# edo01/2024-EUMaster4HPC-Student-Challenge

Measured on AMD Instinct MI355X. Metric: cg_iterations_per_sec, higher is better.
Workload: dtype f64

## Files before the change

### 2024-eumaster4hpc-student-challenge_amd/csrc/lam_ctx.h

```cpp
#pragma once

namespace {

thread_local std::string g_create_error;

double now_s()
{
    return std::chrono::duration<double>(std::chrono::steady_clock::now().time_since_epoch()).count();
}

uint64_t thread_cpu_ns()
{
    struct timespec ts;
    if (clock_gettime(CLOCK_THREAD_CPUTIME_ID, &ts) != 0) return 0;
    return (uint64_t)ts.tv_sec * 1000000000ull + (uint64_t)ts.tv_nsec;
}

constexpr int kLag = 4;
constexpr int64_t kRankModeDefaultExchange = 1;
constexpr int64_t kOneProcessDefaultExchange = 1;
constexpr int kVecBlocksMax = 256;

struct SymvDevPlan {
    SymvTask *tasks = nullptr;
// ... 113 lines not shown
    bool shifted = false;
    MshiftState ms;
    MinresState mr;
    SymvDevPlan sym;
    int sym_vec = 0, sym_cap_K = 0;
};

struct PcgState {
    void *diag = nullptr, *dinv = nullptr;
    double *part_rz = nullptr;
    DiagInfo *info = nullptr;
    uint64_t diag_gen = ~0ull;
    uint64_t bad_count = 0, bad_row = 0;
    double bad_value = 0.0;
    void *dinv_k = nullptr;
    uint64_t dinvk_gen = ~0ull;
    int dinvk_K = 0, dinvk_nrhs = 0;
    double dinvk_shift[kMaxRhs] = {};
    uint64_t badk_count = 0, badk_row = 0;
    int badk_col = 0;
    double badk_value = 0.0;
};

}

struct lam_hip_ctx {
    MultiState multi;
    PcgState pcg;
    int dtype = LAM_HIP_F64;
    int total_shards = 1;
    int rank = 0, nranks = 1;
    bool rank_mode = false;
    ncclComm_t comm = nullptr;
    double t_comm_init = 0.0;
    uint64_t n = 0;
    uint64_t lda = 0;
    bool have_problem = false, have_matrix = false, have_rhs = false, cg_ready = false;
    int k_done = 0;
    std::vector<ShardBase> sh;
    std::string err;
    int64_t opt_gemv_variant = -1;
    int64_t opt_nt = 1;
    int64_t opt_generic = 0;
    int64_t opt_probe_rows = 0;
    int64_t opt_overlap = 1;
    int64_t opt_panel_lo = 0, opt_panel_hi = 0;
    bool gather_pending = false;
    int64_t opt_symmetric_many = 0;
    bool symv_many_effective = false;
    int64_t opt_symmetric = 0;
    int64_t opt_exchange = 0;
// ... 21 lines not shown
    bool direct_ok = false;
    bool cg_direct = false;
    int64_t opt_verify_direct = 1;
    int64_t direct_fallbacks = 0;
    uint32_t epoch = 0;
    uint64_t seq_base = 0, seq_span = 1;
    int *direct_err = nullptr;
    double *agree_buf = nullptr;
    bool cg_exchange1 = false;
    double t_gemv_min = 0.0, t_gemv_max = 0.0;
    int xt_slot = -1;
    int ranks_on_device = 1;
    bool symmetric_from_env = false;
    uint64_t matrix_gen = 0, sym_checked_gen = ~0ull;
    bool sym_refused = false;
    bool told_sym_ineffective = false;

    bool symv_wanted() const
    {
        return n > 0 && !sym_refused && (opt_symmetric >= 2 || (opt_symmetric == 1 && n * n * (uint64_t)esz_a() >= (192ull << 20)));
    }
    bool symv_active() const { return symv_wanted() && !rank_mode && total_shards == 1; }
    bool symv_multi_active() const { return symv_wanted() && exchange1_ok(); }
    uint64_t symv_stride_bytes() const { return (n * esz_v() + 7) / 8 * 8 + 8; }

    bool exchange2_wanted() const { return (rank_mode || total_shards > 1) && opt_exchange == 2 && opt_finalize != 0; }
    bool exchange1_ok() const { return (rank_mode || total_shards > 1) && opt_exchange == 1 && n >= (uint64_t)total_shards; }
    uint64_t ex1_base() const { return n / (uint64_t)total_shards; }
    uint64_t ex1_maxrows() const { return n / (uint64_t)total_shards + n % (uint64_t)total_shards; }
    uint64_t ex1_stride_bytes() const { return (ex1_maxrows() * esz_v() + 7) / 8 * 8 + 8; }

    size_t esz_a() const { return dtype == LAM_HIP_F64 ? 8 : (dtype == LAM_HIP_F32 ? 4 : 2); }
    static uint64_t pitch_for(uint64_t n, size_t ea) { return lam::row_pitch(n, ea); }
    uint64_t ncols_vec() const { const uint64_t v = 16 / esz_a(); return (n + v - 1) / v * v; }
    size_t esz_v() const { return dtype == LAM_HIP_F64 ? 8 : 4; }
};

namespace {

int fail(lam_hip_ctx *c, int code, const char *fmt, ...)
{
    char buf[512];
    va_list ap;
    va_start(ap, fmt);
    vsnprintf(buf, sizeof buf, fmt, ap);
    va_end(ap);
// ... 148 lines not shown
```

### 2024-eumaster4hpc-student-challenge_amd/csrc/lam_hip.hip

```cpp
#include <hip/hip_runtime.h>
#include <rccl/rccl.h>

#include <algorithm>
#include <atomic>
#include <chrono>
#include <cmath>
#include <cstdarg>
#include <cstdio>
#include <cstdlib>
#include <cstring>
#include <memory>
#include <new>
#include <mutex>
#include <string>
#include <type_traits>
#include <vector>

#include <sched.h>
#include <time.h>
#include <unistd.h>

#include "../../include/lam_hip.h"
#include "lam_kernels.h"

// ... 111 lines not shown
        c->t_comm_init = now_s() - t0;
        rc = count_ranks_on_device(c.get());
        if (rc != 0) {
            g_create_error = c->err;
            (void)ncclCommDestroy(c->comm);
            c->comm = nullptr;
            abandon(c.get());
            return rc;
        }
    }
    *out = c.release();
    return 0;
}

void lam_hip_destroy(lam_hip_ctx *c)
{
    if (!c) return;
    for (auto &s : c->sh) {
        (void)hipSetDevice(s.dev);
        if (s.stream) (void)hipStreamSynchronize(s.stream);
    }
    multi_release(c);
    close_direct(c);
    if (c->agree_buf) (void)hipFree(c->agree_buf);
    for (auto &s : c->sh) {
        if (hipSetDevice(s.dev) != hipSuccess) { (void)hipGetLastError(); continue; }
        if (s.mail) { (void)hipFree(s.mail); s.mail = nullptr; }
        if (s.bcast) { (void)hipFree(s.bcast); s.bcast = nullptr; }
    }
    if (c->direct_err) (void)hipHostFree(c->direct_err);
    if (c->comm) (void)ncclCommDestroy(c->comm);
    release_join(c);
    for (auto &s : c->sh) {
        free_shard(s);
        release_handles(s);
    }
    delete c;
}

int lam_hip_set_problem(lam_hip_ctx *c, uint64_t n)
{
    if (!c) return LAM_HIP_EINVAL;
    if (n == 0) return fail(c, LAM_HIP_EINVAL, "n must be > 0");
    if (n < (uint64_t)c->total_shards) return fail(c, LAM_HIP_EINVAL, "n (%llu) smaller than the number of shards", (unsigned long long)n);
    if (n != c->multi.n) multi_release(c);
    c->multi.have_rhs = c->multi.solved = c->multi.ms.valid = c->multi.lz.valid = false;
    multi_clear_shifts(c->multi);
    c->n = n;
    c->iter_est_s = 0.0;
    c->lda = lam_hip_ctx::pitch_for(n, c->esz_a());
    c->problem_gen++;
    c->have_problem = c->have_matrix = c->have_rhs = c->cg_ready = false;
    const size_t ea = c->esz_a(), ev = c->esz_v();
    for (auto &s : c->sh) {
        free_shard(s, c->opt_reuse_matrix != 0);
        partition(n, c->total_shards, s.index, &s.row0, &s.nrows);
        LAMCHK(set_dev(c, s));
        const size_t needA = std::max<size_t>(16, s.nrows * c->lda * ea);
        if (s.A != nullptr && s.A_capacity < needA) { (void)hipFree(s.A); s.A = nullptr; s.A_capacity = 0; }
        if (s.A == nullptr) {
            HIPCHK(c, hipMalloc(&s.A, needA));
            s.A_capacity = needA;
        }
        HIPCHK(c, hipMalloc(&s.p, n * ev + 64));
        HIPCHK(c, hipMalloc(&s.tmp, n * ev + 64));
        void **vecs[] = {&s.Ap, &s.x, &s.r, &s.b};
        for (auto v : vecs) HIPCHK(c, hipMalloc(v, s.nrows * ev + 16));
        s.gemv_blocks = dispatch(c, [&](auto impl) -> int { return decltype(impl)::gemv_grid(c, s.nrows); });
        const int gemv_blocks_max = (int)std::max<uint64_t>(s.nrows, (n + kSymvReduceRows - 1) / kSymvReduceRows) + 1;
        s.vec_blocks = vec_grid(s.nrows);
        HIPCHK(c, hipMalloc((void **)&s.part_gemv, sizeof(double) * (size_t)gemv_blocks_max));
        s.part_gemv_cap = gemv_blocks_max;
        HIPCHK(c, hipMalloc((void **)&s.part_vec, sizeof(double) * kVecBlocksMax));
        HIPCHK(c, hipMalloc((void **)&s.part_aux, sizeof(double) * kVecBlocksMax));
        HIPCHK(c, hipMalloc((void **)&s.gather_a, sizeof(double) * kMaxShards));
// ... 322 lines not shown
    ShardBase &s0 = c->sh[0];
    c->prog_t = 0.0;
    IterTimes times;
    int enq = 0;
    LAMCHK(set_dev(c, s0));
    HIPCHK(c, hipMemcpyAsync(s0.sc_host, s0.sc, sizeof(CgScalars), hipMemcpyDeviceToHost, s0.stream));
    HIPCHK(c, hipStreamSynchronize(s0.stream));
    const bool stopped = s0.sc_host->stop != 0;
    const int k_first = c->k_done + 1;
    for (auto &sh_ : c->sh)
        for (int i = 0; i < kLag; i++) { sh_.timed_slot[i] = false; sh_.nx[i] = 0; }
    if (stopped) {
    } else {
        for (int i = 0; i < iters; i++) {
            const int k = k_first + i;
            const int slot = i % kLag;
            if (i >= kLag) {
                LAMCHK(set_dev(c, s0));
                const int d = lag_check(c, s0, k);
                if (d < 0) return d;
                if (d != 0) break;
                harvest_times(c, slot, &times);
            }
            const double te = now_s();
            LAMCHK(enqueue_iteration(c, k, rel_error, slot));
            c->enqueue_ns += (uint64_t)((now_s() - te) * 1e9);
            enq++;
        }
    }
    if (enq > 0) {
        Progress pr;
        LAMCHK(set_dev(c, s0));
        LAMCHK(await_progress(c, s0, k_first + enq - 1, &pr, true));
    }
    LAMCHK(settle_gather(c));
    LAMCHK(sync_all(c));
    if (*c->direct_err != 0) {
        static const char *what[] = {"", "", "a peer's partial dot product (direct exchange)", "a peer's p slice (direct exchange)",
                                     "the reducer workgroup's broadcast inside the fused update launch (its workgroups were not all resident?)",
                                     "a workgroup's partial inside a launch (reducer workgroup)"};
        const int code = c->direct_err[0];
        return fail(c, LAM_HIP_EHIP, "rank %d: a bounded in-kernel wait expired waiting for %s (code %d; slot %d, expected tag %d:%d, saw %d:%d); "
                                     "the iteration state is no longer valid", c->rank, code >= 2 && code <= 5 ? what[code] : "?", code,
                    c->direct_err[1], c->direct_err[4], c->direct_err[2], c->direct_err[5], c->direct_err[3]);
    }
    if (c->cg_direct && c->rank_mode && c->nranks > 1 && enq > 0) {
// ... 7 lines not shown
    const CgScalars sc = *s0.sc_host;
    c->k_done = sc.iters;
    const double t1 = now_s();
    if (st) {
        memset(st, 0, sizeof *st);
        const int ran = sc.iters - (k_first - 1);
        st->converged = sc.stop != 0;
        st->num_iters = sc.stop ? sc.iters : sc.iters + 1;
        st->rel_err = std::sqrt(sc.rr[sc.iters & 1] / sc.bb);
        st->t_total = t1 - t0;
        st->t_iter = ran > 0 ? (t1 - t0) / ran : 0.0;
        double tmin = 0.0, tmax = 0.0;
        for (size_t j = 0; j < c->sh.size(); j++) {
            if (times.samples[j] == 0) continue;
            const double avg = times.gemv_ms[j] * 1e-3 / times.samples[j];
            tmax = std::max(tmax, avg);
            tmin = tmin == 0.0 ? avg : std::min(tmin, avg);
        }
        c->t_gemv_min = tmin;
        c->t_gemv_max = tmax;
        st->t_gemv = tmax;
        st->t_exchange = times.samples[0] > 0 ? times.xch_ms * 1e-3 / times.samples[0] : 0.0;
        st->t_comm_init = c->t_comm_init;
        st->gemv_bytes = (double)c->esz_a() * (double)s0.nrows * (double)c->n + (double)c->esz_v() * (double)(c->n + s0.nrows);
    }
    (void)enq;
    return 0;
}

int lam_hip_solve(lam_hip_ctx *c, int max_iters, double rel_error, lam_hip_stats *st)
{
    if (!c) return LAM_HIP_EINVAL;
    if (max_iters < 0) return fail(c, LAM_HIP_EINVAL, "max_iters must be >= 0");
    const double t0 = now_s();
    lam_hip_stats local;
    LAMCHK(lam_hip_cg_init(c));
    LAMCHK(lam_hip_cg_iterate(c, max_iters, rel_error, &local));
    if (c->cg_direct && c->opt_verify_direct) {
        double tr = 0.0;
        LAMCHK(lam_hip_true_residual(c, &tr));
        const double slack = c->dtype == LAM_HIP_F64 ? 2.2e-10 : 1e-4;
        if (!(tr <= 10.0 * local.rel_err + slack)) {
            if (c->rank == 0)
                fprintf(stderr, "lam_hip: direct exchange: recomputed residual %.3e does not match the recursive residual %.3e -- "
                                "solving again on the RCCL exchange\n", tr, local.rel_err);
            c->direct_fallbacks++;
            c->opt_exchange = 0;
// ... 36 lines not shown
        HIPCHK(c, hipStreamSynchronize(s.stream));
    }
    return 0;
}

static int gemv_tmp(lam_hip_ctx *c)
{
    return dispatch(c, [&](auto impl) -> int {
        using I = decltype(impl);
        using TV = typename ImplTraits<I>::TV;
        for (auto &s : c->sh) {
            LAMCHK(set_dev(c, s));
            LAMCHK(I::launch_gemv(c, s, (const TV *)s.tmp, (TV *)s.Ap, nullptr, nullptr));
        }
        return 0;
    });
}

int lam_hip_gemv(lam_hip_ctx *c, const void *x_host, void *y_host)
{
    if (!c || !x_host || !y_host) return LAM_HIP_EINVAL;
    if (!c->have_matrix) return fail(c, LAM_HIP_ESTATE, "matrix not set");
    LAMCHK(env_symmetric_check(c));
    const size_t ev = c->esz_v();
    for (auto &s : c->sh) {
        LAMCHK(set_dev(c, s));
        HIPCHK(c, hipMemcpyAsync(s.tmp, x_host, c->n * ev, hipMemcpyHostToDevice, s.stream));
    }
    if (c->symv_active()) {
        LAMCHK(dispatch(c, [&](auto impl) -> int {
            using I = decltype(impl);
            using TV = typename ImplTraits<I>::TV;
            ShardBase &s = c->sh[0];
            LAMCHK(set_dev(c, s));
            return I::launch_symv(c, s, (const TV *)s.tmp, (TV *)s.Ap, nullptr, nullptr);
        }));
    } else {
        LAMCHK(gemv_tmp(c));
    }
    c->cg_ready = false;
    if (c->rank_mode) {
        ShardBase &s = c->sh[0];
        const ncclDataType_t dt = c->dtype == LAM_HIP_F64 ? ncclDouble : ncclFloat;
        HIPCHK(c, hipMemcpyAsync((char *)s.tmp + s.row0 * ev, s.Ap, s.nrows * ev, hipMemcpyDeviceToDevice, s.stream));
        NCCLCHK(c, ncclGroupStart());
        for (int q = 0; q < c->nranks; q++) {
// ... 1 lines not shown
            partition(c->n, c->nranks, q, &r0, &nr);
            char *ptr = (char *)s.tmp + r0 * ev;
            NCCLCHK(c, ncclBroadcast(ptr, ptr, nr, dt, q, c->comm, s.stream));
            c->n_collectives++;
        }
        NCCLCHK(c, ncclGroupEnd());
        HIPCHK(c, hipMemcpyAsync(y_host, s.tmp, c->n * ev, hipMemcpyDeviceToHost, s.stream));
        HIPCHK(c, hipStreamSynchronize(s.stream));
        return 0;
    }
    for (auto &s : c->sh) {
        LAMCHK(set_dev(c, s));
        HIPCHK(c, hipMemcpyAsync((char *)y_host + s.row0 * ev, s.Ap, s.nrows * ev, hipMemcpyDeviceToHost, s.stream));
        HIPCHK(c, hipStreamSynchronize(s.stream));
    }
    return 0;
}

int lam_hip_gemv_only(lam_hip_ctx *c, int reps, double *sec)
{
    if (!c || !sec || reps < 1) return LAM_HIP_EINVAL;
    if (!c->have_matrix) return fail(c, LAM_HIP_ESTATE, "matrix not set");
    LAMCHK(env_symmetric_check(c));
    c->cg_ready = false;
    double worst = 0.0;
    LAMCHK(dispatch(c, [&](auto impl) -> int {
        using I = decltype(impl);
        using TV = typename ImplTraits<I>::TV;
        for (auto &s : c->sh) {
            LAMCHK(set_dev(c, s));
            const uint64_t nrows_saved = s.nrows;
            if (c->opt_probe_rows > 0) s.nrows = std::min<uint64_t>(s.nrows, (uint64_t)c->opt_probe_rows);
            const bool split = c->opt_panel_hi > c->opt_panel_lo;
            const uint64_t lo = (uint64_t)c->opt_panel_lo, hi = (uint64_t)c->opt_panel_hi;
            auto one = [&]() -> int {
                if (c->symv_active()) return I::launch_symv(c, s, (const TV *)s.p, (TV *)s.Ap, s.part_gemv, nullptr);
                if (!split) return I::launch_gemv(c, s, (const TV *)s.p, (TV *)s.Ap, s.part_gemv, nullptr);
                int r1 = I::launch_gemv(c, s, (const TV *)s.p, (TV *)s.Ap, nullptr, nullptr, 1, lo, hi);
                return r1 != 0 ? r1 : I::launch_gemv(c, s, (const TV *)s.p, (TV *)s.Ap, s.part_gemv, nullptr, 2, lo, hi);
            };
            int rc = one();
            if (rc == 0 && hipEventRecord(s.ev_g0[0], s.stream) != hipSuccess) rc = LAM_HIP_EHIP;
            for (int i = 0; i < reps && rc == 0; i++) rc = one();
            if (rc == 0 && hipEventRecord(s.ev_g1[0], s.stream) != hipSuccess) rc = LAM_HIP_EHIP;
            s.nrows = nrows_saved;
            if (rc != 0) return rc == LAM_HIP_EHIP ? fail(c, rc, "hipEventRecord failed in gemv_only") : rc;
// ... 215 lines not shown
    else if (!strcmp(name, "exchange")) { c->opt_exchange = value; c->cg_ready = false; }
    else if (!strcmp(name, "exchange_join")) c->opt_join = value;
    else if (!strcmp(name, "finalize")) {
        if (value == 0 && !kTuningBuild)
            return fail(c, LAM_HIP_EINVAL, "finalize = 0 (separate reduction launches, the round-1 chain) exists in the tuning build only (`make tuning`, "
                                           "load liblam_hip_tuning.so through LAM_HIP_LIB), not in the product library");
        c->opt_finalize = value; c->cg_ready = false;
    }
    else if (!strcmp(name, "upload_staging")) c->opt_upload_staging = value;
    else if (!strcmp(name, "reuse_matrix")) c->opt_reuse_matrix = value;
    else if (!strcmp(name, "fuse_update")) { c->opt_fuse = value; c->cg_ready = false; }
    else if (!strcmp(name, "symmetric")) {
        c->opt_symmetric = value;
        c->symmetric_from_env = false;
        c->sym_refused = false;
        c->cg_ready = false;
    }
    else if (!strcmp(name, "symmetric_many")) {
        if (value < 0 || value > 2)
            return fail(c, LAM_HIP_EINVAL, "symmetric_many = %lld: 0 (general batched product), 1 (symmetric where it pays) or 2 (always, K <= 4)",
                        (long long)value);
        c->opt_symmetric_many = value;
    }
    else if (!strcmp(name, "gemv_timing")) c->opt_gemv_timing = value < 0 ? 0 : value;
    else if (!strcmp(name, "verify_direct")) c->opt_verify_direct = value;
    else if (!strcmp(name, "assume_cus")) { c->opt_assume_cus = value; c->cg_ready = false; }
    else if (!strcmp(name, "panel_lo")) c->opt_panel_lo = value;
    else if (!strcmp(name, "panel_hi")) c->opt_panel_hi = value;
    else return fail(c, LAM_HIP_EINVAL, "unknown option '%s'", name);
    for (auto &s : c->sh)
        if (c->have_problem) s.gemv_blocks = dispatch(c, [&](auto impl) -> int { return decltype(impl)::gemv_grid(c, s.nrows); });
    return 0;
}

int lam_hip_get_option(const lam_hip_ctx *c, const char *name, int64_t *value)
{
    if (!c || !name || !value) return LAM_HIP_EINVAL;
    if (!strcmp(name, "gemv_variant")) *value = c->opt_gemv_variant;
    else if (!strcmp(name, "nt_loads")) *value = c->opt_nt;
    else if (!strcmp(name, "force_generic")) *value = c->opt_generic;
    else if (!strcmp(name, "probe_rows")) *value = c->opt_probe_rows;
    else if (!strcmp(name, "overlap")) *value = c->opt_overlap;
    else if (!strcmp(name, "exchange")) *value = c->opt_exchange;
    else if (!strcmp(name, "exchange_join")) *value = c->opt_join;
    else if (!strcmp(name, "finalize")) *value = c->opt_finalize;
    else if (!strcmp(name, "upload_staging")) *value = c->opt_upload_staging;
// ... 3 lines not shown
    else if (!strcmp(name, "rccl_ranks")) {
        int count = 0;
        if (c->comm != nullptr && ncclCommCount(c->comm, &count) != ncclSuccess) count = -1;
        *value = count;
    }
    else if (!strcmp(name, "ranks_on_device")) *value = c->ranks_on_device;
    else if (!strcmp(name, "gemv_ns_min_shard")) *value = (int64_t)(c->t_gemv_min * 1e9);
    else if (!strcmp(name, "gemv_ns_max_shard")) *value = (int64_t)(c->t_gemv_max * 1e9);
    else if (!strcmp(name, "tuning_variants")) *value = kTuningBuild ? 1 : 0;
    else if (!strcmp(name, "fuse_effective")) *value = c->fuse_active ? 1 : 0;
    else if (!strcmp(name, "gemv_timing")) *value = c->opt_gemv_timing;
    else if (!strcmp(name, "verify_direct")) *value = c->opt_verify_direct;
    else if (!strcmp(name, "direct_fallbacks")) *value = c->direct_fallbacks;
    else if (!strcmp(name, "assume_cus")) *value = c->opt_assume_cus;
    else if (!strcmp(name, "host_enqueue_ns")) *value = (int64_t)c->enqueue_ns;
    else if (!strcmp(name, "host_cpu_ns")) *value = (int64_t)c->host_cpu_ns;
    else if (!strcmp(name, "row_pitch")) *value = (int64_t)c->lda;
    else if (!strcmp(name, "hip_calls_launch")) *value = (int64_t)c->n_launch;
    else if (!strcmp(name, "hip_calls_record")) *value = (int64_t)c->n_record;
    else if (!strcmp(name, "hip_calls_wait")) *value = (int64_t)c->n_wait;
    else if (!strcmp(name, "hip_calls_setdevice")) *value = (int64_t)c->n_setdev;
    else if (!strcmp(name, "symmetric")) *value = c->opt_symmetric;
    else if (!strcmp(name, "symmetric_many")) *value = c->opt_symmetric_many;
    else if (!strcmp(name, "symmetric_many_effective")) *value = c->symv_many_effective ? 1 : 0;
    else if (!strcmp(name, "symmetric_effective")) *value = (c->symv_active() || c->symv_multi_active()) ? 1 : 0;
    else if (!strcmp(name, "exchange_effective")) *value = c->cg_direct ? 2 : ((c->exchange1_ok() && !c->exchange2_wanted()) ? 1 : 0);
    else if (!strcmp(name, "panel_lo")) *value = c->opt_panel_lo;
    else if (!strcmp(name, "panel_hi")) *value = c->opt_panel_hi;
    else if (!strcmp(name, "multi_rhs_k")) *value = c->multi.last_K;
    else if (!strcmp(name, "deflation_m")) *value = deflate_valid(c) ? c->multi.df.m : 0;
    else return LAM_HIP_EINVAL;
    return 0;
}

}
```

### 2024-eumaster4hpc-student-challenge_amd/csrc/lam_kernels.h

```cpp
#pragma once

#include <hip/hip_runtime.h>
#include <hip/hip_bf16.h>
#include <stdint.h>

#include <limits>
#include <type_traits>

#include "lam_host_plan.h"
#include "lam_host_tridiag.h"
#include "lam_host_chol.h"
#include "lam_host_block.h"

namespace lam {

constexpr int kBlock = 256;
constexpr int kWaves = kBlock / 64;
__device__ __attribute__((aligned(16))) const unsigned int kZeroVec16[4] = {0u, 0u, 0u, 0u};
constexpr int kMaxShards = 64;
constexpr size_t kAgreeBytes = 256 * (size_t)kMaxShards;

struct CgScalars {
    double bb;
    double rr[2];
    double pAp;
    double alpha;
    double beta;
    int iters;
    int stop;
};

template <typename T>
// ... 532 lines not shown
                TV pv[VEC];
#pragma unroll
                for (int i = 0; i < VEC; i++) pv[i] = s_p[col + i];
#pragma unroll
                for (int r = 0; r < R; r++)
#pragma unroll
                    for (int i = 0; i < VEC; i++) acc[r] = fma_tv((TV)MV::get(av[r], i), pv[i], acc[r]);
            }
        }
        tt = (tt + 1 == ntiles) ? 0 : tt + 1;
    }

#pragma unroll
    for (int r = 0; r < R; r++) {
        TV s = wave_sum(acc[r]);
        if (lane == 0) s_part[r][wave] = s;
    }
    __syncthreads();
    if (tid < R) {
        const uint64_t row = row_first + tid;
        double d = 0.0;
        if (row < a.nrows) {
            TV s = s_part[tid][0];
#pragma unroll
            for (int w = 1; w < WAVES; w++) s += s_part[tid][w];
            if (a.accumulate) s += a.y[row];
            store_y(a, row, s);
            d = (double)s * (double)a.p[a.row0 + row];
        }
        s_dot[tid] = d;
    }
    if (a.partial != nullptr) {
        __syncthreads();
        double t = 0.0;
        if (tid == 0) {
            t = s_dot[0];
#pragma unroll
            for (int r = 1; r < R; r++) t += s_dot[r];
        }
        publish_partial(t, a.partial, a.fin);
    }
}

#ifdef LAM_TUNING_VARIANTS
typedef __bf16 mfma_bf16x8 __attribute__((ext_vector_type(8)));
typedef float mfma_f32x16 __attribute__((ext_vector_type(16)));
// ... 2862 lines not shown
```

### 2024-eumaster4hpc-student-challenge_amd/csrc/lam_launch.h

```cpp
#pragma once

namespace {

Finalize no_finalize(const lam_hip_ctx *c)
{
    Finalize f;
    f.active = 0;
    f.mail = 0;
    f.seq = 0;
    f.dst.n = 0;
    f.slot = 0;
    f.host_err = c ? c->direct_err : nullptr;
    return f;
}

template <typename TA, typename TV>
struct Impl {
    static constexpr int VEC = MatVec<TA>::N;

    static bool variant_available(int v)
    {
        switch (v) {
        case 0: case 10: case 13: case 17: return true;
#ifdef LAM_TUNING_VARIANTS
// ... 7 lines not shown
        switch (v) {
        case 0: return 16;
        case 17: return 4;
        case 20: return 8;
        case 21: return 16;
        default: return 2;
        }
    }

    static bool fast_ok(const lam_hip_ctx *c) { return !c->opt_generic; }
    static int variant(const lam_hip_ctx *c)
    {
        if (c->opt_gemv_variant >= 0 && variant_available((int)c->opt_gemv_variant)) return (int)c->opt_gemv_variant;
        return sizeof(TA) == 2 ? 0 : (sizeof(TA) == 8 ? 13 : 10);
    }

    static std::string kernel_name(const lam_hip_ctx *c)
    {
        const char *ta = sizeof(TA) == 8 ? "double" : (sizeof(TA) == 4 ? "float" : "__hip_bfloat16");
        const char *tv = sizeof(TV) == 8 ? "double" : "float";
        char buf[192];
        if (c->symv_active()) { snprintf(buf, sizeof buf, "symv_task_kernel<%s,NV=1> + symv_reduce_kernel<%s,NV=1>", ta, ta); return buf; }
        if (!fast_ok(c)) { snprintf(buf, sizeof buf, "gemv_generic_kernel<%s,%s>", ta, tv); return buf; }
        const int v = variant(c);
        const char *nt = c->opt_nt ? "true" : "false";
        if (v == 0) snprintf(buf, sizeof buf, "gemv_tile_kernel<%s,%s,R=4,TILE=4096,NT=%s,UNROLL=4,LDS=true,ROT=true>", ta, tv, nt);
        else if (v >= 20) snprintf(buf, sizeof buf, "gemv_mfma_bf16_kernel<R=%d,TILE=4096,NT=true,SPLIT=%d>", v == 20 ? 2 : 4, v == 20 ? 1 : 3);
        else
            snprintf(buf, sizeof buf, "gemv_coop_kernel<%s,%s,R=%d,TILE=4096,NT=%s,UNROLL=4,WAVES=%d>", ta, tv, variant_rows_per_block(v), nt,
                     v == 10 ? 4 : 8);
        return buf;
    }

    static int gemv_grid(const lam_hip_ctx *c, uint64_t nrows)
    {
        if (nrows == 0) return 0;
        if (c->symv_active()) return symv_reduce_grid(c->n);
        return kernel_grid(c, nrows);
    }

    static int kernel_grid(const lam_hip_ctx *c, uint64_t nrows)
    {
        if (nrows == 0) return 0;
        const uint64_t rows_per_block = fast_ok(c) ? (uint64_t)variant_rows_per_block(variant(c)) : (uint64_t)kWaves;
        return (int)((nrows + rows_per_block - 1) / rows_per_block);
    }
// ... 45 lines not shown
    {
        if (s.nrows == 0) return 0;
        GemvArgs<TA, TV> a;
        a.A = (const TA *)s.A; a.p = p; a.y = y; a.partial = partial; a.sc = sc;
        a.n_ypeer = 0;
        for (auto &yp : a.ypeer) yp = nullptr;
        if (ypeers != nullptr)
            for (int j = 0; j < ypeers->n && a.n_ypeer < kMaxShards - 1; j++) a.ypeer[a.n_ypeer++] = (TV *)ypeers->p[j];
        a.fin = (fin != nullptr && partial != nullptr) ? *fin : no_finalize(c);
        a.nrows = s.nrows; a.n = c->n; a.row0 = s.row0; a.lda = c->lda;
        const uint64_t ncols = fast_ok(c) ? c->ncols_vec() : c->n;
        if (fast_ok(c) && hi == c->n) hi = ncols;
        a.seg_begin[0] = 0; a.seg_end[0] = ncols; a.seg_begin[1] = a.seg_end[1] = 0; a.nseg = 1; a.accumulate = 0;
        if (panel == 1) { a.seg_begin[0] = lo; a.seg_end[0] = hi; }
        else if (panel == 2) {
            a.accumulate = 1;
            a.nseg = 0;
            if (lo > 0) { a.seg_begin[a.nseg] = 0; a.seg_end[a.nseg] = lo; a.nseg++; }
            if (hi < ncols) { a.seg_begin[a.nseg] = hi; a.seg_end[a.nseg] = ncols; a.nseg++; }
            if (a.nseg == 0) return 0;
            if (a.nseg == 1) { a.seg_begin[1] = a.seg_end[1] = 0; }
        }
        const int grid = kernel_grid(c, s.nrows) + (a.fin.active ? 1 : 0);
        if (fast_ok(c)) {
            switch (variant(c)) {
            default:
            case 0: launch_tile(c, grid, s.stream, a); break;
            case 10: launch_coop<2, 4>(c, grid, s.stream, a); break;
            case 13: launch_coop<2, 8>(c, grid, s.stream, a); break;
            case 17: launch_coop<4, 8>(c, grid, s.stream, a); break;
#ifdef LAM_TUNING_VARIANTS
            case 20: case 21:
                if constexpr (sizeof(TA) == 2) {
                    if (variant(c) == 20) hipLaunchKernelGGL((gemv_mfma_bf16_kernel<2, 4096, true, 1>), dim3(grid), dim3(kBlock), 0, s.stream, a);
                    else hipLaunchKernelGGL((gemv_mfma_bf16_kernel<4, 4096, true, 3>), dim3(grid), dim3(kBlock), 0, s.stream, a);
                }
                break;
#endif
            }
        } else {
            hipLaunchKernelGGL((gemv_generic_kernel<TA, TV>), dim3(grid), dim3(kBlock), 0, s.stream, a);
        }
        LAUNCHED(c);
        return 0;
    }
};

template <typename T> struct ImplTraits;
template <typename TA_, typename TV_> struct ImplTraits<Impl<TA_, TV_>> { using TA = TA_; using TV = TV_; };

template <typename I>
void cg_panel(const lam_hip_ctx *c, const ShardBase &s, uint64_t *lo, uint64_t *hi)
{
    *lo = *hi = 0;
    uint64_t a = 0, b = 0;
    if (c->opt_panel_hi > c->opt_panel_lo) { a = (uint64_t)c->opt_panel_lo; b = std::min<uint64_t>((uint64_t)c->opt_panel_hi, c->n); }
    else if (c->rank_mode && c->opt_overlap && c->nranks > 1) { a = s.row0; b = s.row0 + s.nrows; }
    if (b <= a || (a == 0 && b >= c->n)) return;
    if (I::fast_ok(c) && (a % I::VEC != 0 || (b % I::VEC != 0 && b != c->n))) return;
    *lo = a; *hi = b;
}

template <typename F>
int dispatch(lam_hip_ctx *c, F &&f)
{
    switch (c->dtype) {
    case LAM_HIP_F64: return f(Impl<double, double>());
    case LAM_HIP_F32: return f(Impl<float, float>());
    case LAM_HIP_BF16: return f(Impl<__hip_bfloat16, float>());
// ... 81 lines not shown
```

Before: 208.1.

## Add lossless 7-byte packed f64 matrix format with packed GEMV kernel

Adds a device kernel that re-encodes each 4096-column tile of the f64 matrix into 7 bytes per element. Each tile gets a shared exponent window, and values outside that window are stored as exceptions in a side array. A matching packed GEMV kernel decodes on the fly. Packing is triggered automatically after a number of plain products when the matrix is at least 8 GiB and there is enough free memory, so the memory-bound GEMV streams fewer bytes. The trade-offs are a one-time packing pass, extra device memory, decode ALU work and exception lookups through LDS.

```diff
diff --git a/2024-eumaster4hpc-student-challenge_amd/csrc/lam_ctx.h b/2024-eumaster4hpc-student-challenge_amd/csrc/lam_ctx.h
--- a/2024-eumaster4hpc-student-challenge_amd/csrc/lam_ctx.h
+++ b/2024-eumaster4hpc-student-challenge_amd/csrc/lam_ctx.h
@@ -159,11 +159,27 @@
     double badk_value = 0.0;
 };
 
+constexpr int kPackAfter = 65;
+constexpr uint64_t kPackMinBytes = 8ull << 30;
+struct PackState {
+    void *buf = nullptr;
+    size_t cap = 0;
+    uint64_t nrows = 0, ntiles = 0;
+    uint64_t ready_gen = ~0ull;
+    uint64_t refused_gen = ~0ull;
+    uint64_t count_gen = ~0ull;
+    uint64_t plain = 0;
+    uint64_t exc_total = 0;
+    double pack_s = 0.0;
+};
+
 }
 
 struct lam_hip_ctx {
     MultiState multi;
     PcgState pcg;
+    PackState pack;
+    int64_t opt_packed = -1;
     int dtype = LAM_HIP_F64;
     int total_shards = 1;
     int rank = 0, nranks = 1;
@@ -231,6 +247,12 @@
     }
     bool symv_active() const { return symv_wanted() && !rank_mode && total_shards == 1; }
     bool symv_multi_active() const { return symv_wanted() && exchange1_ok(); }
+    bool pack_eligible() const
+    {
+        return opt_packed != 0 && dtype == LAM_HIP_F64 && !rank_mode && total_shards == 1 && opt_symmetric == 0 && opt_generic == 0 &&
+               opt_gemv_variant < 0 && n > 0;
+    }
+    bool pack_active() const { return pack_eligible() && pack.buf != nullptr && pack.ready_gen == matrix_gen; }
     uint64_t symv_stride_bytes() const { return (n * esz_v() + 7) / 8 * 8 + 8; }
 
     bool exchange2_wanted() const { return (rank_mode || total_shards > 1) && opt_exchange == 2 && opt_finalize != 0; }
diff --git a/2024-eumaster4hpc-student-challenge_amd/csrc/lam_hip.hip b/2024-eumaster4hpc-student-challenge_amd/csrc/lam_hip.hip
--- a/2024-eumaster4hpc-student-challenge_amd/csrc/lam_hip.hip
+++ b/2024-eumaster4hpc-student-challenge_amd/csrc/lam_hip.hip
@@ -157,6 +157,7 @@
     }
     multi_release(c);
     close_direct(c);
+    if (c->pack.buf && !c->sh.empty() && hipSetDevice(c->sh[0].dev) == hipSuccess) (void)hipFree(c->pack.buf);
     if (c->agree_buf) (void)hipFree(c->agree_buf);
     for (auto &s : c->sh) {
         if (hipSetDevice(s.dev) != hipSuccess) { (void)hipGetLastError(); continue; }
@@ -186,6 +187,7 @@
     c->lda = lam_hip_ctx::pitch_for(n, c->esz_a());
     c->problem_gen++;
     c->have_problem = c->have_matrix = c->have_rhs = c->cg_ready = false;
+    c->pack.ready_gen = c->pack.refused_gen = c->pack.count_gen = ~0ull;
     const size_t ea = c->esz_a(), ev = c->esz_v();
     for (auto &s : c->sh) {
         free_shard(s, c->opt_reuse_matrix != 0);
@@ -554,6 +556,7 @@
                 if (d != 0) break;
                 harvest_times(c, slot, &times);
             }
+            LAMCHK(pack_maybe(c));
             const double te = now_s();
             LAMCHK(enqueue_iteration(c, k, rel_error, slot));
             c->enqueue_ns += (uint64_t)((now_s() - te) * 1e9);
@@ -607,7 +610,7 @@
         st->t_gemv = tmax;
         st->t_exchange = times.samples[0] > 0 ? times.xch_ms * 1e-3 / times.samples[0] : 0.0;
         st->t_comm_init = c->t_comm_init;
-        st->gemv_bytes = (double)c->esz_a() * (double)s0.nrows * (double)c->n + (double)c->esz_v() * (double)(c->n + s0.nrows);
+        st->gemv_bytes = gemv_bytes_now(c, s0);
     }
     (void)enq;
     return 0;
@@ -690,6 +693,7 @@
     if (!c || !x_host || !y_host) return LAM_HIP_EINVAL;
     if (!c->have_matrix) return fail(c, LAM_HIP_ESTATE, "matrix not set");
     LAMCHK(env_symmetric_check(c));
+    LAMCHK(pack_maybe(c));
     const size_t ev = c->esz_v();
     for (auto &s : c->sh) {
         LAMCHK(set_dev(c, s));
@@ -737,6 +741,7 @@
     if (!c || !sec || reps < 1) return LAM_HIP_EINVAL;
     if (!c->have_matrix) return fail(c, LAM_HIP_ESTATE, "matrix not set");
     LAMCHK(env_symmetric_check(c));
+    LAMCHK(pack_maybe(c));
     c->cg_ready = false;
     double worst = 0.0;
     LAMCHK(dispatch(c, [&](auto impl) -> int {
@@ -998,6 +1003,11 @@
                         (long long)value);
         c->opt_symmetric_many = value;
     }
+    else if (!strcmp(name, "packed")) {
+        if (value < -1 || value > 1)
+            return fail(c, LAM_HIP_EINVAL, "packed = %lld: -1 (automatic), 0 (never) or 1 (pack in front of the next product)", (long long)value);
+        c->opt_packed = value;
+    }
     else if (!strcmp(name, "gemv_timing")) c->opt_gemv_timing = value < 0 ? 0 : value;
     else if (!strcmp(name, "verify_direct")) c->opt_verify_direct = value;
     else if (!strcmp(name, "assume_cus")) { c->opt_assume_cus = value; c->cg_ready = false; }
@@ -1047,6 +1057,10 @@
     else if (!strcmp(name, "hip_calls_setdevice")) *value = (int64_t)c->n_setdev;
     else if (!strcmp(name, "symmetric")) *value = c->opt_symmetric;
     else if (!strcmp(name, "symmetric_many")) *value = c->opt_symmetric_many;
+    else if (!strcmp(name, "packed")) *value = c->opt_packed;
+    else if (!strcmp(name, "packed_effective")) *value = c->pack_active() ? 1 : 0;
+    else if (!strcmp(name, "packed_bytes")) *value = c->pack_active() ? (int64_t)gemv_bytes_now(c, c->sh[0]) : 0;
+    else if (!strcmp(name, "packed_pack_ns")) *value = c->pack_active() ? (int64_t)(c->pack.pack_s * 1e9) : 0;
     else if (!strcmp(name, "symmetric_many_effective")) *value = c->symv_many_effective ? 1 : 0;
     else if (!strcmp(name, "symmetric_effective")) *value = (c->symv_active() || c->symv_multi_active()) ? 1 : 0;
     else if (!strcmp(name, "exchange_effective")) *value = c->cg_direct ? 2 : ((c->exchange1_ok() && !c->exchange2_wanted()) ? 1 : 0);
diff --git a/2024-eumaster4hpc-student-challenge_amd/csrc/lam_host_pack.h b/2024-eumaster4hpc-student-challenge_amd/csrc/lam_host_pack.h
--- /dev/null
+++ b/2024-eumaster4hpc-student-challenge_amd/csrc/lam_host_pack.h
@@ -0,0 +1,141 @@
+#pragma once
+
+#include <stdint.h>
+
+#include <cstddef>
+#include <cstring>
+
+#if defined(__HIPCC__)
+#define LAM_HOST_DEVICE __host__ __device__ __forceinline__
+#else
+#define LAM_HOST_DEVICE inline
+#endif
+
+namespace lam {
+
+constexpr uint32_t kPackTile = 4096;
+constexpr uint32_t kPackGroups = 8;
+constexpr uint32_t kPackGroupBytes = 3584;
+constexpr uint32_t kPackTileBytes = kPackGroups * kPackGroupBytes;
+constexpr uint32_t kPackWindow = 7;
+constexpr uint32_t kPackCap = 256;
+constexpr uint32_t kPackZeroIdx = kPackCap;
+constexpr uint32_t kPackFirst = 64;
+constexpr uint32_t kPackExpBins = 2048;
+
+LAM_HOST_DEVICE void pack_pos(uint32_t j, uint32_t *w, uint32_t *l, uint32_t *e)
+{
+    *w = (j >> 7) & 7u;
+    *l = (j & 127u) >> 1;
+    *e = 2u * (j >> 10) + (j & 1u);
+}
+LAM_HOST_DEVICE uint32_t pack_off_lo(uint32_t l, uint32_t e) { return (e >> 2) * 1024u + l * 16u + (e & 3u) * 4u; }
+LAM_HOST_DEVICE uint32_t pack_off_mid(uint32_t l, uint32_t e) { return 2048u + l * 16u + e * 2u; }
+LAM_HOST_DEVICE uint32_t pack_off_hi(uint32_t l, uint32_t e) { return 3072u + l * 8u + e; }
+
+LAM_HOST_DEVICE uint32_t pack_exp_of(uint64_t bits) { return (uint32_t)(bits >> 52) & 0x7ffu; }
+LAM_HOST_DEVICE bool pack_is_normal(uint64_t bits) { const uint32_t x = pack_exp_of(bits); return x >= 1u && x <= 2046u; }
+LAM_HOST_DEVICE bool pack_in_window(uint64_t bits, uint32_t base)
+{
+    const uint32_t x = pack_exp_of(bits);
+    return x >= 1u && x <= 2046u && x <= base && base - x < kPackWindow;
+}
+LAM_HOST_DEVICE uint32_t pack_window_count(const uint32_t *hist, uint32_t base)
+{
+    uint32_t c = 0;
+    for (uint32_t k = 0; k < kPackWindow; k++)
+        if (base >= 1u + k && base - k <= 2046u) c += hist[base - k];
+    return c;
+}
+LAM_HOST_DEVICE uint32_t pack_window_key(uint32_t count, uint32_t base) { return count << 11 | base; }
+
+LAM_HOST_DEVICE void pack_encode(uint64_t bits, uint32_t base, uint32_t *lo, uint32_t *mid, uint32_t *hi)
+{
+    const uint32_t field = 6u - (base - pack_exp_of(bits));
+    const uint32_t t = field << 21 | ((uint32_t)(bits >> 32) & 0xfffffu) << 1 | (uint32_t)(bits >> 63);
+    *lo = (uint32_t)bits;
+    *mid = t & 0xffffu;
+    *hi = t >> 16;
+}
+LAM_HOST_DEVICE void pack_encode_exception(uint32_t index, uint32_t *lo, uint32_t *mid, uint32_t *hi)
+{
+    *lo = index;
+    *mid = 0u;
+    *hi = 7u << 5;
+}
+LAM_HOST_DEVICE bool pack_is_exception(uint32_t t) { return t >= 7u << 21; }
+LAM_HOST_DEVICE uint32_t pack_exp_shift(uint32_t base) { return (base - 6u) << 20; }
+LAM_HOST_DEVICE uint64_t pack_decode(uint32_t lo, uint32_t t, uint32_t exp_shift)
+{
+    const uint32_t hw = ((t >> 1) + exp_shift) | t << 31;
+    return (uint64_t)hw << 32 | lo;
+}
+
+LAM_HOST_DEVICE uint32_t pack_header(uint32_t base, uint32_t count) { return base | (count > 0xffffu ? 0xffffu : count) << 16; }
+LAM_HOST_DEVICE uint32_t pack_header_base(uint32_t h) { return h & 0x7ffu; }
+LAM_HOST_DEVICE uint32_t pack_header_count(uint32_t h) { return h >> 16; }
+
+struct PackLayout { size_t data, exc, hdr, total; };
+inline PackLayout pack_layout(uint64_t nrows, uint64_t ntiles)
+{
+    auto up = [](size_t v) { return (v + 255) / 256 * 256; };
+    PackLayout L;
+    L.data = 0;
+    L.exc = up((size_t)nrows * ntiles * kPackTileBytes);
+    L.hdr = L.exc + up((size_t)nrows * ntiles * kPackCap * 8);
+    L.total = L.hdr + up((size_t)nrows * ntiles * 4);
+    return L;
+}
+
+#if !defined(__HIP_DEVICE_COMPILE__)
+inline uint32_t pack_tile(const uint64_t *in, uint32_t cols, unsigned char *data, uint64_t *exc, uint32_t *header)
+{
+    uint32_t hist[kPackExpBins];
+    memset(hist, 0, sizeof hist);
+    for (uint32_t j = 0; j < cols; j++)
+        if (pack_is_normal(in[j])) hist[pack_exp_of(in[j])]++;
+    uint32_t best = 0;
+    for (uint32_t base = 1; base <= 2046u; base++) {
+        const uint32_t key = pack_window_key(pack_window_count(hist, base), base);
+        if (key > best) best = key;
+    }
+    const uint32_t base = best & 0x7ffu;
+    uint32_t count = 0;
+    for (uint32_t j = 0; j < kPackTile; j++) {
+        uint32_t w, l, e, lo, mid, hi;
+        pack_pos(j, &w, &l, &e);
+        if (j >= cols) pack_encode_exception(kPackZeroIdx, &lo, &mid, &hi);
+        else if (pack_in_window(in[j], base)) pack_encode(in[j], base, &lo, &mid, &hi);
+        else {
+            if (count < kPackCap) exc[count] = in[j];
+            pack_encode_exception(count < kPackCap ? count : kPackZeroIdx, &lo, &mid, &hi);
+            count++;
+        }
+        unsigned char *g = data + (size_t)w * kPackGroupBytes;
+        const uint16_t m16 = (uint16_t)mid;
+        memcpy(g + pack_off_lo(l, e), &lo, 4);
+        memcpy(g + pack_off_mid(l, e), &m16, 2);
+        g[pack_off_hi(l, e)] = (unsigned char)hi;
+    }
+    *header = pack_header(base, count);
+    return count;
+}
+
+inline void unpack_tile(const unsigned char *data, const uint64_t *exc, uint32_t header, uint64_t *out)
+{
+    const uint32_t base = pack_header_base(header);
+    for (uint32_t j = 0; j < kPackTile; j++) {
+        uint32_t w, l, e, lo;
+        uint16_t m16;
+        pack_pos(j, &w, &l, &e);
+        const unsigned char *g = data + (size_t)w * kPackGroupBytes;
+        memcpy(&lo, g + pack_off_lo(l, e), 4);
+        memcpy(&m16, g + pack_off_mid(l, e), 2);
+        const uint32_t t = (uint32_t)g[pack_off_hi(l, e)] << 16 | m16;
+        if (pack_is_exception(t)) out[j] = lo < kPackCap ? exc[lo] : 0ull;
+        else out[j] = pack_decode(lo, t, pack_exp_shift(base));
+    }
+}
+#endif
+
+}
diff --git a/2024-eumaster4hpc-student-challenge_amd/csrc/lam_kernels.h b/2024-eumaster4hpc-student-challenge_amd/csrc/lam_kernels.h
--- a/2024-eumaster4hpc-student-challenge_amd/csrc/lam_kernels.h
+++ b/2024-eumaster4hpc-student-challenge_amd/csrc/lam_kernels.h
@@ -8,6 +8,7 @@
 #include <type_traits>
 
 #include "lam_host_plan.h"
+#include "lam_host_pack.h"
 #include "lam_host_tridiag.h"
 #include "lam_host_chol.h"
 #include "lam_host_block.h"
@@ -586,6 +587,251 @@
         double d = 0.0;
         if (row < a.nrows) {
             TV s = s_part[tid][0];
+#pragma unroll
+            for (int w = 1; w < WAVES; w++) s += s_part[tid][w];
+            if (a.accumulate) s += a.y[row];
+            store_y(a, row, s);
+            d = (double)s * (double)a.p[a.row0 + row];
+        }
+        s_dot[tid] = d;
+    }
+    if (a.partial != nullptr) {
+        __syncthreads();
+        double t = 0.0;
+        if (tid == 0) {
+            t = s_dot[0];
+#pragma unroll
+            for (int r = 1; r < R; r++) t += s_dot[r];
+        }
+        publish_partial(t, a.partial, a.fin);
+    }
+}
+
+struct PackedMat {
+    const unsigned char *data;
+    const double *exc;
+    const uint32_t *hdr;
+    uint32_t ntiles;
+};
+typedef unsigned int pack_u4 __attribute__((ext_vector_type(4)));
+typedef unsigned int pack_u2 __attribute__((ext_vector_type(2)));
+
+__global__ void __launch_bounds__(kBlock)
+pack_rows_kernel(const double *__restrict__ A, uint64_t lda, uint64_t ncols, uint32_t ntiles, unsigned char *__restrict__ data,
+                 uint64_t *__restrict__ exc, uint32_t *__restrict__ hdr, unsigned long long *__restrict__ info)
+{
+    typedef double dvec2 __attribute__((ext_vector_type(2)));
+    __shared__ uint32_t s_hist[kPackExpBins];
+    __shared__ uint32_t s_key[kWaves];
+    __shared__ uint32_t s_cnt;
+    __shared__ uint64_t s_exc[kPackCap];
+
+    const int tid = threadIdx.x, lane = tid & 63, wave = tid >> 6;
+    const uint64_t row = blockIdx.x;
+    const double *arow = A + row * lda;
+    unsigned long long row_exc = 0;
+    for (uint32_t tt = 0; tt < ntiles; tt++) {
+        const uint64_t c0 = (uint64_t)tt * kPackTile;
+        const uint32_t cols = (uint32_t)((ncols - c0 < (uint64_t)kPackTile) ? (ncols - c0) : (uint64_t)kPackTile);
+        for (int i = tid; i < (int)kPackExpBins; i += kBlock) s_hist[i] = 0;
+        if (tid == 0) s_cnt = 0;
+        __syncthreads();
+        uint64_t v[2][8];
+        uint32_t valid = 0;
+#pragma unroll
+        for (int h = 0; h < 2; h++)
+#pragma unroll
+            for (int s = 0; s < 4; s++) {
+                const uint32_t col = (uint32_t)s * 1024u + (uint32_t)(wave + 4 * h) * 128u + 2u * (uint32_t)lane;
+                v[h][2 * s] = v[h][2 * s + 1] = 0;
+                if (col < cols) {
+                    const dvec2 a = __builtin_nontemporal_load(reinterpret_cast<const dvec2 *>(arow + c0 + col));
+                    v[h][2 * s] = (uint64_t)__double_as_longlong(a[0]);
+                    v[h][2 * s + 1] = (uint64_t)__double_as_longlong(a[1]);
+                    valid |= 1u << (4 * h + s);
+                }
+            }
+#pragma unroll
+        for (int h = 0; h < 2; h++)
+#pragma unroll
+            for (int e = 0; e < 8; e++)
+                if ((valid >> (4 * h + (e >> 1)) & 1u) && pack_is_normal(v[h][e])) atomicAdd(&s_hist[pack_exp_of(v[h][e])], 1u);
+        __syncthreads();
+        uint32_t key = 0;
+        for (uint32_t base = (uint32_t)tid * 8u; base < (uint32_t)tid * 8u + 8u; base++)
+            if (base >= 1u && base <= 2046u) key = max(key, pack_window_key(pack_window_count(s_hist, base), base));
+#pragma unroll
+        for (int off = 32; off > 0; off >>= 1) key = max(key, (uint32_t)__shfl_xor((int)key, off, 64));
+        if (lane == 0) s_key[wave] = key;
+        __syncthreads();
+        key = s_key[0];
+#pragma unroll
+        for (int w = 1; w < kWaves; w++) key = max(key, s_key[w]);
+        const uint32_t base = key & 0x7ffu;
+
+        const uint64_t unit = row * ntiles + tt;
+#pragma unroll
+        for (int h = 0; h < 2; h++) {
+            uint32_t lo[8], mid[8], hi[8];
+#pragma unroll
+            for (int e = 0; e < 8; e++) {
+                if (!(valid >> (4 * h + (e >> 1)) & 1u)) pack_encode_exception(kPackZeroIdx, &lo[e], &mid[e], &hi[e]);
+                else if (pack_in_window(v[h][e], base)) pack_encode(v[h][e], base, &lo[e], &mid[e], &hi[e]);
+                else {
+                    const uint32_t idx = atomicAdd(&s_cnt, 1u);
+                    if (idx < kPackCap) s_exc[idx] = v[h][e];
+                    pack_encode_exception(idx < kPackCap ? idx : kPackZeroIdx, &lo[e], &mid[e], &hi[e]);
+                }
+            }
+            unsigned char *g = data + (unit * kPackGroups + (uint64_t)(wave + 4 * h)) * kPackGroupBytes;
+            pack_u4 q;
+            q[0] = lo[0]; q[1] = lo[1]; q[2] = lo[2]; q[3] = lo[3];
+            *reinterpret_cast<pack_u4 *>(g + pack_off_lo(lane, 0)) = q;
+            q[0] = lo[4]; q[1] = lo[5]; q[2] = lo[6]; q[3] = lo[7];
+            *reinterpret_cast<pack_u4 *>(g + pack_off_lo(lane, 4)) = q;
+            q[0] = mid[0] | mid[1] << 16; q[1] = mid[2] | mid[3] << 16; q[2] = mid[4] | mid[5] << 16; q[3] = mid[6] | mid[7] << 16;
+            *reinterpret_cast<pack_u4 *>(g + pack_off_mid(lane, 0)) = q;
+            pack_u2 b;
+            b[0] = hi[0] | hi[1] << 8 | hi[2] << 16 | hi[3] << 24;
+            b[1] = hi[4] | hi[5] << 8 | hi[6] << 16 | hi[7] << 24;
+            *reinterpret_cast<pack_u2 *>(g + pack_off_hi(lane, 0)) = b;
+        }
+        __syncthreads();
+        const uint32_t cnt = s_cnt;
+        for (uint32_t i = tid; i < cnt && i < kPackCap; i += kBlock) exc[unit * kPackCap + i] = s_exc[i];
+        if (tid == 0) {
+            hdr[unit] = pack_header(base, cnt);
+            row_exc += max(min(cnt, kPackCap), kPackFirst);
+            if (cnt > kPackCap) info[0] = 1ull;
+        }
+        __syncthreads();
+    }
+    if (tid == 0) atomicAdd(&info[1], row_exc);
+}
+
+template <bool NT>
+__global__ void __launch_bounds__(512)
+gemv_packed_kernel(GemvArgs<double, double> a, PackedMat pk)
+{
+    constexpr int R = 2, WAVES = 8, TILE = kPackTile, STEP = 128, NTHREADS = WAVES * 64;
+    constexpr int WSTEPS = TILE / (STEP * WAVES);
+    static_assert(WSTEPS == 4 && STEP * WAVES == 1024, "the packed layout is that of 8 waves x 4 super-steps");
+
+    __shared__ __attribute__((aligned(16))) double s_p[TILE];
+    __shared__ double s_exc[R][kPackCap + 1];
+    __shared__ double s_part[R][WAVES];
+    __shared__ double s_dot[R];
+    __shared__ double s_red[kWaves];
+
+    if (a.sc != nullptr && a.sc->stop) return;
+    if (is_reducer_block(a.fin)) { reduce_partials(a.partial, (int)gridDim.x - 1, a.fin, s_red); return; }
+
+    const int tid = threadIdx.x;
+    const int lane = tid & 63;
+    const int wave = __builtin_amdgcn_readfirstlane(tid >> 6);
+    const uint64_t row_first = (uint64_t)blockIdx.x * R;
+    const uint32_t woff = (uint32_t)wave * STEP + (uint32_t)lane * 2u;
+
+    const uint32_t ntiles = pk.ntiles;
+    uint64_t unit0[R];
+#pragma unroll
+    for (int r = 0; r < R; r++) {
+        uint64_t row = row_first + r;
+        if (row >= a.nrows) row = a.nrows - 1;
+        unit0[r] = row * ntiles;
+    }
+    double acc[R];
+#pragma unroll
+    for (int r = 0; r < R; r++) acc[r] = 0.0;
+    if (tid < R) s_exc[tid][kPackZeroIdx] = 0.0;
+
+    constexpr uint32_t FIRST = kPackFirst;
+    static_assert(FIRST == 64, "one value a lane");
+    static_assert(R <= WAVES - 1, "waves 1 .. R stage the lists' first values");
+    const bool stager = wave >= 1 && wave <= R;
+    uint32_t perlane = 0;
+    asm volatile("" : "+v"(perlane));
+    uint32_t tt = blockIdx.x % ntiles;
+    for (uint32_t t = 0; t < ntiles; t++) {
+        const uint64_t c0 = (uint64_t)tt * TILE;
+        const uint64_t cend = a.seg_end[0];
+        const uint32_t cols = (uint32_t)((cend - c0 < (uint64_t)TILE) ? (cend - c0) : (uint64_t)TILE);
+        const uint32_t tnext = (tt + 1 == ntiles) ? 0 : tt + 1;
+        pack_u4 lo0[R], lo1[R], mid[R];
+        pack_u2 hi[R];
+#pragma unroll
+        for (int r = 0; r < R; r++) {
+            const unsigned char *g = pk.data + ((unit0[r] + tt) * kPackGroups + (uint64_t)wave) * kPackGroupBytes;
+            const pack_u4 *q0 = reinterpret_cast<const pack_u4 *>(g + pack_off_lo(lane, 0));
+            const pack_u4 *q1 = reinterpret_cast<const pack_u4 *>(g + pack_off_lo(lane, 4));
+            const pack_u4 *qm = reinterpret_cast<const pack_u4 *>(g + pack_off_mid(lane, 0));
+            const pack_u2 *qh = reinterpret_cast<const pack_u2 *>(g + pack_off_hi(lane, 0));
+            lo0[r] = NT ? __builtin_nontemporal_load(q0) : *q0;
+            lo1[r] = NT ? __builtin_nontemporal_load(q1) : *q1;
+            mid[r] = NT ? __builtin_nontemporal_load(qm) : *qm;
+            hi[r] = NT ? __builtin_nontemporal_load(qh) : *qh;
+        }
+        uint32_t head[R];
+#pragma unroll
+        for (int r = 0; r < R; r++) head[r] = pk.hdr[unit0[r] + tt + perlane];
+        double first = 0.0;
+        if (stager) first = pk.exc[(unit0[wave - 1] + tt) * kPackCap + lane];
+        __syncthreads();
+        {
+            typedef double pvec_t __attribute__((ext_vector_type(2)));
+            const pvec_t *src = reinterpret_cast<const pvec_t *>(a.p + c0);
+            pvec_t *dst = reinterpret_cast<pvec_t *>(s_p);
+            const uint32_t nv = cols / 2;
+            for (uint32_t i = tid; i < nv; i += NTHREADS) dst[i] = src[i];
+            for (uint32_t i = nv * 2 + tid; i < cols; i += NTHREADS) s_p[i] = a.p[c0 + i];
+            for (uint32_t i = cols + tid; i < (uint32_t)TILE && i < (cols + STEP * WAVES - 1) / (STEP * WAVES) * (STEP * WAVES); i += NTHREADS)
+                s_p[i] = 0.0;
+        }
+        uint32_t shift[R];
+#pragma unroll
+        for (int r = 0; r < R; r++) {
+            shift[r] = pack_exp_shift(pack_header_base(head[r]));
+            if (stager && wave == 1 + r) s_exc[r][lane] = first;
+            const uint32_t cnt = min(pack_header_count(head[r]), kPackCap);
+            const double *e = pk.exc + (unit0[r] + tt) * kPackCap;
+            for (uint32_t i = FIRST + tid; i < cnt; i += NTHREADS) s_exc[r][i] = e[i];
+        }
+        __syncthreads();
+        const int nsteps = (int)((cols + STEP * WAVES - 1) / (STEP * WAVES));
+#pragma unroll
+        for (int s = 0; s < WSTEPS; s++) {
+            if (s < nsteps) {
+                double pv[2];
+#pragma unroll
+                for (int i = 0; i < 2; i++) pv[i] = s_p[s * (STEP * WAVES) + woff + i];
+#pragma unroll
+                for (int r = 0; r < R; r++)
+#pragma unroll
+                    for (int i = 0; i < 2; i++) {
+                        const int e = 2 * s + i;
+                        const uint32_t l = e < 4 ? lo0[r][e & 3] : lo1[r][e & 3];
+                        const uint32_t w = ((hi[r][e >> 2] >> (8 * (e & 3))) & 0xffu) << 16 | ((mid[r][e >> 1] >> (16 * (e & 1))) & 0xffffu);
+                        const bool x = pack_is_exception(w);
+                        const double ev = s_exc[r][x ? min(l, kPackZeroIdx) : kPackZeroIdx];
+                        const double av = x ? ev : __longlong_as_double((long long)pack_decode(l, w, shift[r]));
+                        acc[r] = fma_tv(av, pv[i], acc[r]);
+                    }
+            }
+        }
+        tt = tnext;
+    }
+
+#pragma unroll
+    for (int r = 0; r < R; r++) {
+        double s = wave_sum(acc[r]);
+        if (lane == 0) s_part[r][wave] = s;
+    }
+    __syncthreads();
+    if (tid < R) {
+        const uint64_t row = row_first + tid;
+        double d = 0.0;
+        if (row < a.nrows) {
+            double s = s_part[tid][0];
 #pragma unroll
             for (int w = 1; w < WAVES; w++) s += s_part[tid][w];
             if (a.accumulate) s += a.y[row];
diff --git a/2024-eumaster4hpc-student-challenge_amd/csrc/lam_launch.h b/2024-eumaster4hpc-student-challenge_amd/csrc/lam_launch.h
--- a/2024-eumaster4hpc-student-challenge_amd/csrc/lam_launch.h
+++ b/2024-eumaster4hpc-student-challenge_amd/csrc/lam_launch.h
@@ -53,6 +53,10 @@
         char buf[192];
         if (c->symv_active()) { snprintf(buf, sizeof buf, "symv_task_kernel<%s,NV=1> + symv_reduce_kernel<%s,NV=1>", ta, ta); return buf; }
         if (!fast_ok(c)) { snprintf(buf, sizeof buf, "gemv_generic_kernel<%s,%s>", ta, tv); return buf; }
+        if (c->pack_active()) {
+            snprintf(buf, sizeof buf, "gemv_packed_kernel<double,double,R=2,TILE=4096,NT=%s,WAVES=8>", c->opt_nt ? "true" : "false");
+            return buf;
+        }
         const int v = variant(c);
         const char *nt = c->opt_nt ? "true" : "false";
         if (v == 0) snprintf(buf, sizeof buf, "gemv_tile_kernel<%s,%s,R=4,TILE=4096,NT=%s,UNROLL=4,LDS=true,ROT=true>", ta, tv, nt);
@@ -144,6 +148,25 @@
             if (a.nseg == 1) { a.seg_begin[1] = a.seg_end[1] = 0; }
         }
         const int grid = kernel_grid(c, s.nrows) + (a.fin.active ? 1 : 0);
+        if constexpr (sizeof(TA) == 8) {
+            if (panel == 0 && c->pack_eligible()) {
+                PackState &pk = c->pack;
+                if (c->pack_active() && s.nrows <= pk.nrows) {
+                    const PackLayout L = pack_layout(pk.nrows, pk.ntiles);
+                    PackedMat m;
+                    m.data = (const unsigned char *)pk.buf + L.data;
+                    m.exc = (const double *)((const char *)pk.buf + L.exc);
+                    m.hdr = (const uint32_t *)((const char *)pk.buf + L.hdr);
+                    m.ntiles = (uint32_t)pk.ntiles;
+                    if (c->opt_nt) hipLaunchKernelGGL((gemv_packed_kernel<true>), dim3(grid), dim3(512), 0, s.stream, a, m);
+                    else hipLaunchKernelGGL((gemv_packed_kernel<false>), dim3(grid), dim3(512), 0, s.stream, a, m);
+                    LAUNCHED(c);
+                    return 0;
+                }
+                if (pk.count_gen != c->matrix_gen) { pk.count_gen = c->matrix_gen; pk.plain = 0; }
+                pk.plain++;
+            }
+        }
         if (fast_ok(c)) {
             switch (variant(c)) {
             default:
@@ -167,6 +190,66 @@
         return 0;
     }
 };
+
+int set_dev(lam_hip_ctx *c, const ShardBase &s);
+int pack_maybe(lam_hip_ctx *c)
+{
+    if (!c->pack_eligible() || !c->have_matrix) return 0;
+    PackState &pk = c->pack;
+    if (pk.ready_gen == c->matrix_gen || pk.refused_gen == c->matrix_gen) return 0;
+    ShardBase &s = c->sh[0];
+    const bool automatic = c->opt_packed < 0;
+    if (automatic) {
+        if (pk.count_gen != c->matrix_gen || pk.plain < (uint64_t)kPackAfter) return 0;
+        if (s.nrows * c->lda * 8ull < kPackMinBytes) return 0;
+    }
+    const uint64_t ncols = c->ncols_vec();
+    const uint64_t ntiles = (ncols + kPackTile - 1) / kPackTile;
+    const PackLayout L = pack_layout(s.nrows, ntiles);
+    const size_t need = L.total + 256;
+    LAMCHK(set_dev(c, s));
+    if (pk.cap < need) {
+        if (automatic) {
+            size_t free_b = 0, total_b = 0;
+            if (hipMemGetInfo(&free_b, &total_b) != hipSuccess) { (void)hipGetLastError(); free_b = 0; }
+            if (free_b + pk.cap < 2 * need) { pk.refused_gen = c->matrix_gen; return 0; }
+        }
+        HIPCHK(c, hipStreamSynchronize(s.stream));
+        if (pk.buf != nullptr) { (void)hipFree(pk.buf); pk.buf = nullptr; pk.cap = 0; }
+        if (hipMalloc(&pk.buf, need) != hipSuccess) {
+            (void)hipGetLastError();
+            pk.buf = nullptr;
+            pk.refused_gen = c->matrix_gen;
+            return 0;
+        }
+        pk.cap = need;
+    }
+    pk.ready_gen = ~0ull;
+    pk.nrows = s.nrows; pk.ntiles = ntiles;
+    unsigned long long *info = (unsigned long long *)((char *)pk.buf + L.total);
+    unsigned long long got[2] = {0, 0};
+    HIPCHK(c, hipStreamSynchronize(s.stream));
+    const double t0 = now_s();
+    HIPCHK(c, hipMemsetAsync(info, 0, 16, s.stream));
+    hipLaunchKernelGGL(pack_rows_kernel, dim3((unsigned)s.nrows), dim3(kBlock), 0, s.stream, (const double *)s.A, c->lda, ncols, (uint32_t)ntiles,
+                       (unsigned char *)pk.buf + L.data, (uint64_t *)((char *)pk.buf + L.exc), (uint32_t *)((char *)pk.buf + L.hdr), info);
+    HIPCHK(c, hipGetLastError());
+    HIPCHK(c, hipMemcpyAsync(got, info, 16, hipMemcpyDeviceToHost, s.stream));
+    HIPCHK(c, hipStreamSynchronize(s.stream));
+    pk.pack_s = now_s() - t0;
+    if (got[0] != 0) { pk.refused_gen = c->matrix_gen; return 0; }
+    pk.exc_total = got[1];
+    pk.ready_gen = c->matrix_gen;
+    return 0;
+}
+
+double gemv_bytes_now(const lam_hip_ctx *c, const ShardBase &s0)
+{
+    const double vec = (double)c->esz_v() * (double)(c->n + s0.nrows);
+    if (!c->pack_active()) return (double)c->esz_a() * (double)s0.nrows * (double)c->n + vec;
+    const double units = (double)s0.nrows * (double)c->pack.ntiles;
+    return units * (double)(kPackTileBytes + 4) + 8.0 * (double)c->pack.exc_total + vec;
+}
 
 template <typename T> struct ImplTraits;
 template <typename TA_, typename TV_> struct ImplTraits<Impl<TA_, TV_>> { using TA = TA_; using TV = TV_; };
```

After: 219.7 (median of 6 runs). 1.06x the previous value.
